# nanoporetech/medaka

Measured on NVIDIA H100. Metric: pileup positions/sec (consensus inference), higher is better.
Workload: dtype f32

## Files before the change

medaka_b200/csrc/gru_wg.cu:

```cuda
#include "common.cuh"
#include "ptx.cuh"
#include "rec_common.cuh"

namespace mdk {

constexpr int RW_THREADS = 256;
constexpr int RW_ABLK = (H / 8) * 64 * 16;
constexpr int RW_XBLK = 2 * 64 * 16;

template <int NT, bool FUSE_X, int OUT>
struct RwCfg {
    static constexpr int N = NT * RT_N;
    static constexpr bool HL = NT == 1;
    static constexpr int ROWS = HL ? 2 * N : N;
    static constexpr int PLANES = HL ? 1 : 2;
    static constexpr int KG = ROWS * 16 + 16;
    static constexpr int HPLANE = (H / 8) * KG;
    static constexpr int XPLANE = 2 * KG;
    static constexpr int HLO = HL ? N * 16 : HPLANE;
    static constexpr int XLO = HL ? N * 16 : XPLANE;
    static constexpr int RED = (RW_THREADS / 32) * NCLS * N;
    static constexpr int wlo_off = 0;
    static constexpr int wxlo_off = wlo_off + 6 * RW_ABLK;
    static constexpr int h_off = wxlo_off + (FUSE_X ? 6 * RW_XBLK : 0);
    static constexpr int x_off = h_off + 2 * PLANES * HPLANE;
    static constexpr int red_off = x_off + (FUSE_X ? 2 * PLANES * XPLANE : 0);
    static constexpr int total = red_off + (OUT == OUT_LOGITS ? 2 * RED * 4 : 0);
    static_assert(total <= 227 * 1024, "smem budget");
};

__device__ __forceinline__ uint32_t ld_u32(const __half *p) { return *reinterpret_cast<const uint32_t *>(p); }

template <int NT, bool FUSE_X, int OUT>
__global__ void __launch_bounds__(RW_THREADS, 1)
rec_tc_kernel(const float *__restrict__ gi, RecX xin, const __half *__restrict__ w_hh, const float *__restrict__ b_hn,
              void *__restrict__ h_out, int64_t B, int64_t T, const float *__restrict__ lin_w,
              float *__restrict__ plog) {
    using L = RwCfg<NT, FUSE_X, OUT>;
    constexpr int N = L::N, NA = N / 2;
    constexpr int NACC = L::ROWS / 2;
    constexpr int NX = FUSE_X ? NACC : NA;
    using MMA = Wgmma<N>;
    using MMA_H = Wgmma<L::ROWS>;
    constexpr bool LOGITS = OUT == OUT_LOGITS;
    extern __shared__ __align__(128) uint8_t smem[];
    const int tid = threadIdx.x, wg = tid >> 7, warp = (tid >> 5) & 3, lane = tid & 31;
    const int gq = lane >> 2, cq = lane & 3;
    const int dir = blockIdx.y;
    const int64_t ntiles = (B + RT_N - 1) / RT_N;
    const int64_t wtile0 = (int64_t)blockIdx.x * NT;
    const int j0 = wg * 64 + warp * 16 + gq;
    const uint32_t sbase = smem_u32(smem);

    for (int i = tid; i < (L::total - L::h_off) / 16; i += RW_THREADS)
        reinterpret_cast<int4 *>(smem + L::h_off)[i] = make_int4(0, 0, 0, 0);
    for (int i = tid; i < 3 * H * (H / 8); i += RW_THREADS) {
        const int kg = i & 15, r = (i >> 4) & (H - 1), gate = i >> 11;
        const uint4 v = *reinterpret_cast<const uint4 *>(w_hh + ((((size_t)dir * 2 + 1) * 3 + gate) * H + r) * H + kg * 8);
        *reinterpret_cast<uint4 *>(smem + L::wlo_off + (gate * 2 + (r >> 6)) * RW_ABLK + kg * 1024 + (r & 63) * 16) = v;
    }
    if (FUSE_X) {
        for (int i = tid; i < 3 * H * 2; i += RW_THREADS) {
            const int kg = i & 1, r = (i >> 1) & (H - 1), gate = i >> 8;
            const uint4 v = *reinterpret_cast<const uint4 *>(xin.w_x + ((((size_t)dir * 2 + 1) * 3 + gate) * H + r) * 16 + kg * 8);
            *reinterpret_cast<uint4 *>(smem + L::wxlo_off + (gate * 2 + (r >> 6)) * RW_XBLK + kg * 1024 + (r & 63) * 16) = v;
        }
    }
    float wlin[2][NCLS];
    if (LOGITS) {
#pragma unroll
        for (int hb = 0; hb < 2; ++hb)
#pragma unroll
            for (int c = 0; c < NCLS; ++c) wlin[hb][c] = lin_w[c * H2 + dir * H + j0 + 8 * hb];
    }
    uint32_t whi[3][H / 16][4];
#pragma unroll
    for (int gate = 0; gate < 3; ++gate)
#pragma unroll
        for (int ks = 0; ks < H / 16; ++ks) {
            const __half *w = w_hh + ((((size_t)dir * 2) * 3 + gate) * H + j0) * H + ks * 16 + 2 * cq;
            whi[gate][ks][0] = ld_u32(w);
            whi[gate][ks][1] = ld_u32(w + 8 * H);
            whi[gate][ks][2] = ld_u32(w + 8);
            whi[gate][ks][3] = ld_u32(w + 8 * H + 8);
        }
    uint32_t wxhi[3][4];
    float bx[3][2] = {};
    if (FUSE_X) {
#pragma unroll
        for (int gate = 0; gate < 3; ++gate) {
            const __half *w = xin.w_x + ((((size_t)dir * 2) * 3 + gate) * H + j0) * 16 + 2 * cq;
            wxhi[gate][0] = ld_u32(w);
            wxhi[gate][1] = ld_u32(w + 8 * 16);
            wxhi[gate][2] = ld_u32(w + 8);
            wxhi[gate][3] = ld_u32(w + 8 * 16 + 8);
            bx[gate][0] = xin.bias[dir * G3 + gate * H + j0];
            bx[gate][1] = xin.bias[dir * G3 + gate * H + j0 + 8];
        }
    }
    const float bhn[2] = {b_hn[dir * H + j0], b_hn[dir * H + j0 + 8]};

    float ar[NACC], az[NACC], an[NACC], axn[NX], hp[NA];
#pragma unroll
    for (int k = 0; k < NA; ++k) hp[k] = 0.f;
    auto load_pre = [&](int64_t t) {
#pragma unroll
        for (int i = 0; i < N / 8; ++i)
#pragma unroll
            for (int hb = 0; hb < 2; ++hb) {
                float2 v[3] = {make_float2(0.f, 0.f), make_float2(0.f, 0.f), make_float2(0.f, 0.f)};
                if (FUSE_X) {
#pragma unroll
                    for (int gate = 0; gate < 3; ++gate) v[gate] = make_float2(bx[gate][hb], bx[gate][hb]);
                } else if (wtile0 + (i >> 1) < ntiles) {
                    const float *p = gi + ((wtile0 + (i >> 1)) * T + t) * GI_TS_FLOATS +
                                     (((dir * 3) * 4 + 2 * (i & 1) + (cq >> 1)) * H + j0 + 8 * hb) * 4 + 2 * (cq & 1);
#pragma unroll
                    for (int gate = 0; gate < 3; ++gate) v[gate] = __ldcs(reinterpret_cast<const float2 *>(p + gate * 16 * H));
                }
                const int k = 4 * i + 2 * hb;
                ar[k] = v[0].x; ar[k + 1] = v[0].y;
                az[k] = v[1].x; az[k + 1] = v[1].y;
                axn[k] = v[2].x; axn[k + 1] = v[2].y;
                an[k] = bhn[hb]; an[k + 1] = bhn[hb];
            }
        if constexpr (L::HL) {
#pragma unroll
            for (int k = NA; k < NACC; ++k) {
                ar[k] = 0.f; az[k] = 0.f; an[k] = 0.f;
                if constexpr (FUSE_X) axn[k] = 0.f;
            }
        }
    };
    const int xF = FUSE_X ? xin.F : 1;
    const float *xsrc[NT];
    int xoff[NT];
    float xreg[NT];
#pragma unroll
    for (int m = 0; m < NT; ++m) {
        const int q = tid + RW_THREADS * m, xn = q / xF, xf = q - xn * xF;
        const bool own = FUSE_X && q < N * xF;
        xoff[m] = own ? (xf >> 3) * L::KG + xn * 16 + (xf & 7) * 2 : -1;
        xsrc[m] = (own && wtile0 * RT_N + xn < B) ? xin.feats + ((wtile0 * RT_N + xn) * T) * xF + xf : nullptr;
        xreg[m] = 0.f;
    }
    auto stage_x = [&](int buf, int m, float v) {
        __half hi, lo;
        split_f16(v, hi, lo);
        *reinterpret_cast<__half *>(smem + L::x_off + buf * L::PLANES * L::XPLANE + xoff[m]) = hi;
        *reinterpret_cast<__half *>(smem + L::x_off + buf * L::PLANES * L::XPLANE + L::XLO + xoff[m]) = lo;
    };
    const int64_t t_first = dir ? T - 1 : 0;
    if (FUSE_X) {
#pragma unroll
        for (int m = 0; m < NT; ++m) {
            if (xoff[m] < 0) continue;
            stage_x(0, m, xsrc[m] ? xsrc[m][t_first * xF] : 0.f);
            if (xsrc[m] && T > 1) xreg[m] = xsrc[m][(dir ? T - 2 : 1) * xF];
        }
    }
    load_pre(t_first);
    fence_proxy_async_smem();
    __syncthreads();

    constexpr int NW = N / 4;
    auto head_partials = [&](int rb) {
        float v[NW][NCLS];
#pragma unroll
        for (int wl = 0; wl < NW; ++wl) {
            const int k = 4 * (wl >> 1) + (wl & 1);
#pragma unroll
            for (int c = 0; c < NCLS; ++c) v[wl][c] = fmaf(wlin[1][c], hp[k + 2], wlin[0][c] * hp[k]);
        }
        int wbase = 0;
#pragma unroll
        for (int lvl = 0; lvl < 3; ++lvl) {
            const int mask = 16 >> lvl;
            const int half = (NW >> lvl) / 2;
            if (half > 0) {
                const bool up = lane & mask;
#pragma unroll
                for (int w = 0; w < NW / 2; ++w) {
                    if (w >= half) continue;
#pragma unroll
                    for (int c = 0; c < NCLS; ++c) {
                        const float send = up ? v[w][c] : v[w + half][c];
                        const float keep = up ? v[w + half][c] : v[w][c];
                        v[w][c] = keep + __shfl_xor_sync(0xffffffffu, send, mask);
                    }
                }
                if (up) wbase += half;
            } else {
#pragma unroll
                for (int c = 0; c < NCLS; ++c) v[0][c] += __shfl_xor_sync(0xffffffffu, v[0][c], mask);
            }
        }
        if (NW >= 8 || !(lane & 4)) {
            float *red = reinterpret_cast<float *>(smem + L::red_off) + rb * L::RED + (tid >> 5) * NCLS * N;
            const int n = 8 * (wbase >> 1) + 2 * cq + (wbase & 1);
#pragma unroll
            for (int c = 0; c < NCLS; ++c) red[c * N + n] = v[0][c];
        }
    };
    auto head_store = [&](int rb, int64_t t) {
        if (tid >= NCLS * N) return;
        const int c = tid / N, n = tid % N;
        const float *red = reinterpret_cast<const float *>(smem + L::red_off) + rb * L::RED + c * N + n;
        float s = red[0];
#pragma unroll
        for (int w = 1; w < RW_THREADS / 32; ++w) s += red[w * NCLS * N];
        const int64_t wt = wtile0 + n / RT_N;
        if (wt < ntiles) plog[((dir * ntiles + wt) * T + t) * PLOG_TS_FLOATS + c * RT_N + (n & 15)] = s;
    };

#pragma unroll 1
    for (int64_t step = 0; step < T; ++step) {
        const int64_t t = dir ? T - 1 - step : step;
        const int buf = (int)(step & 1);
        const uint32_t hb_addr = sbase + L::h_off + buf * L::PLANES * L::HPLANE;
        wg_fence();
        if constexpr (L::HL) {
#pragma unroll
            for (int ks = 0; ks < H / 16; ++ks) {
                const uint64_t bh = make_smem_desc(hb_addr + ks * 2 * L::KG, L::KG, 128);
#pragma unroll
                for (int gate = 0; gate < 3; ++gate) MMA_H::rs(gate == 0 ? ar : (gate == 1 ? az : an), whi[gate][ks], bh, 1u);
#pragma unroll
                for (int gate = 0; gate < 3; ++gate)
                    MMA::ss(gate == 0 ? ar : (gate == 1 ? az : an),
                            make_smem_desc(sbase + L::wlo_off + (gate * 2 + wg) * RW_ABLK + ks * 2 * 1024, 1024, 128), bh, 1u);
            }
        } else {
#pragma unroll
            for (int gate = 0; gate < 3; ++gate) {
                float(&acc)[NACC] = gate == 0 ? ar : (gate == 1 ? az : an);
#pragma unroll
                for (int ks = 0; ks < H / 16; ++ks) {
                    const uint64_t bh = make_smem_desc(hb_addr + ks * 2 * L::KG, L::KG, 128);
                    MMA::rs(acc, whi[gate][ks], bh, 1u);
                    MMA::rs(acc, whi[gate][ks], make_smem_desc(hb_addr + L::HPLANE + ks * 2 * L::KG, L::KG, 128), 1u);
                    MMA::ss(acc, make_smem_desc(sbase + L::wlo_off + (gate * 2 + wg) * RW_ABLK + ks * 2 * 1024, 1024, 128), bh, 1u);
                }
            }
        }
        if constexpr (FUSE_X) {
            const uint32_t xa = sbase + L::x_off + buf * L::PLANES * L::XPLANE;
            const uint64_t bh = make_smem_desc(xa, L::KG, 128);
            if constexpr (L::HL) {
#pragma unroll
                for (int gate = 0; gate < 3; ++gate) MMA_H::rs(gate == 0 ? ar : (gate == 1 ? az : axn), wxhi[gate], bh, 1u);
#pragma unroll
                for (int gate = 0; gate < 3; ++gate)
                    MMA::ss(gate == 0 ? ar : (gate == 1 ? az : axn),
                            make_smem_desc(sbase + L::wxlo_off + (gate * 2 + wg) * RW_XBLK, 1024, 128), bh, 1u);
            } else {
                const uint64_t bl = make_smem_desc(xa + L::XPLANE, L::KG, 128);
#pragma unroll
                for (int gate = 0; gate < 3; ++gate) {
                    float(&acc)[NACC] = gate == 0 ? ar : (gate == 1 ? az : axn);
                    MMA::rs(acc, wxhi[gate], bh, 1u);
                    MMA::rs(acc, wxhi[gate], bl, 1u);
                    MMA::ss(acc, make_smem_desc(sbase + L::wxlo_off + (gate * 2 + wg) * RW_XBLK, 1024, 128), bh, 1u);
                }
            }
        }
        wg_commit();
        if (!FUSE_X && tid == 0 && step + GI_PREFETCH_STEPS < T) {
            const int64_t tp = dir ? t - GI_PREFETCH_STEPS : t + GI_PREFETCH_STEPS;
#pragma unroll
            for (int m = 0; m < NT; ++m) {
                if (wtile0 + m >= ntiles) break;
                const float *blk = gi + ((wtile0 + m) * T + tp) * GI_TS_FLOATS + (int64_t)dir * (GI_TS_FLOATS / 2);
#pragma unroll
                for (int i = 0; i < 12; ++i) bulk_prefetch_l2(blk + i * 512, 2048);
            }
        }
        if (LOGITS && step > 0) {
            if (step > 1) head_store((int)((step - 1) & 1), dir ? t + 2 : t - 2);
            head_partials((int)(step & 1));
        }
        wg_wait_all();
        wg_hold(ar); wg_hold(az); wg_hold(an); wg_hold(axn);

        uint8_t *hw = smem + L::h_off + (buf ^ 1) * L::PLANES * L::HPLANE;
#pragma unroll
        for (int k = 0; k < NA; ++k) {
            float pr = ar[k], pz = az[k], pn = an[k], px = axn[k], r, z;
            if constexpr (L::HL) {
                pr += ar[k + NA]; pz += az[k + NA]; pn += an[k + NA];
                if constexpr (FUSE_X) px += axn[k + NA];
                const float a = 1.f + ex2_approx(fminf(pr, EXP_CLAMP)), b = 1.f + ex2_approx(fminf(pz, EXP_CLAMP));
                const float q = rcp_approx(a * b);
                r = b * q;
                z = a * q;
            } else {
                r = rcp_approx(1.f + ex2_approx(fminf(pr, EXP_CLAMP)));
                z = rcp_approx(1.f + ex2_approx(fminf(pz, EXP_CLAMP)));
            }
            const float en = ex2_approx(fminf(fmaf(r, pn, px), EXP_CLAMP));
            const float n = (en - 1.f) * rcp_approx(en + 1.f);
            hp[k] = fmaf(z, hp[k] - n, n);
            const int j = j0 + 8 * ((k >> 1) & 1), col = 8 * (k >> 2) + 2 * cq + (k & 1);
            __half hi, lo;
            split_f16(hp[k], hi, lo);
            *reinterpret_cast<__half *>(hw + (j >> 3) * L::KG + col * 16 + (j & 7) * 2) = hi;
            *reinterpret_cast<__half *>(hw + L::HLO + (j >> 3) * L::KG + col * 16 + (j & 7) * 2) = lo;
        }
        if (FUSE_X && step + 1 < T) {
#pragma unroll
            for (int m = 0; m < NT; ++m) {
                if (xoff[m] < 0) continue;
                stage_x(buf ^ 1, m, xreg[m]);
                if (xsrc[m] && step + 2 < T) xreg[m] = xsrc[m][(dir ? t - 2 : t + 2) * xF];
            }
        }
        if (!LOGITS) {
#pragma unroll
            for (int k = 0; k < NA; ++k) {
                const int i = k >> 2, n = 8 * i + 2 * cq + (k & 1);
                const int64_t wt = wtile0 + (i >> 1);
                if (wt >= ntiles) continue;
                const int64_t orow = (wt * T + t) * RT_N + (n & 15);
                const int kcol = dir * H + j0 + 8 * ((k >> 1) & 1);
                if (OUT == OUT_TILES) {
                    __half hi, lo;
                    split_f16(hp[k], hi, lo);
                    __half *o = reinterpret_cast<__half *>(reinterpret_cast<uint8_t *>(h_out) + (orow >> 7) * (int64_t)XT_TILE_BYTES +
                                                           (kcol >> 3) * (XT_ROWS * 16) + (orow & (XT_ROWS - 1)) * 16) + (kcol & 7);
                    o[0] = hi;
                    o[XT_PLANE_BYTES / 2] = lo;
                } else {
                    reinterpret_cast<float *>(h_out)[orow * H2 + kcol] = hp[k];
                }
            }
        }
        if (step + 1 < T) load_pre(dir ? t - 1 : t + 1);
        fence_proxy_async_smem();
        __syncthreads();
    }
    if (LOGITS) {
        if (T > 1) head_store((int)((T - 1) & 1), dir ? 1 : T - 2);
        head_partials((int)(T & 1));
        __syncthreads();
        head_store((int)(T & 1), dir ? 0 : T - 1);
    }
}

template <int NT, bool FX, int OUT>
static cudaError_t launch_rec(const float *gi, const RecX &xin, const __half *w_hh_tm, const float *b_hn, void *out,
                              const float *lin_w, int64_t B, int64_t T, cudaStream_t s) {
    auto kern = rec_tc_kernel<NT, FX, OUT>;
    constexpr int smem_bytes = RwCfg<NT, FX, OUT>::total;
    cudaError_t e = cudaFuncSetAttribute(kern, cudaFuncAttributeMaxDynamicSharedMemorySize, smem_bytes);
    if (e != cudaSuccess) return e;
    const int64_t tiles = (B + RT_N - 1) / RT_N;
    dim3 grid((unsigned)((tiles + NT - 1) / NT), NDIR);
    constexpr bool LOGITS = OUT == OUT_LOGITS;
    kern<<<grid, RW_THREADS, smem_bytes, s>>>(gi, xin, w_hh_tm, b_hn, LOGITS ? nullptr : out, B, T, lin_w,
                                              LOGITS ? static_cast<float *>(out) : nullptr);
    return cudaGetLastError();
}

template <int NT>
static cudaError_t launch_rec_nt(const float *gi, const RecX *xin, const __half *w_hh_tm, const float *b_hn, int out_kind,
                                 void *out, const float *lin_w, int64_t B, int64_t T, cudaStream_t s) {
    if (xin)
        return out_kind == OUT_TILES ? launch_rec<NT, true, OUT_TILES>(gi, *xin, w_hh_tm, b_hn, out, nullptr, B, T, s)
                                     : cudaErrorInvalidValue;
    const RecX none{nullptr, nullptr, nullptr, 0};
    switch (out_kind) {
    case OUT_TILES: return launch_rec<NT, false, OUT_TILES>(gi, none, w_hh_tm, b_hn, out, nullptr, B, T, s);
    case OUT_ROWS: return launch_rec<NT, false, OUT_ROWS>(gi, none, w_hh_tm, b_hn, out, nullptr, B, T, s);
    case OUT_LOGITS:
        return lin_w ? launch_rec<NT, false, OUT_LOGITS>(gi, none, w_hh_tm, b_hn, out, lin_w, B, T, s) : cudaErrorInvalidValue;
    }
    return cudaErrorInvalidValue;
}

cudaError_t launch_rec_tc(const float *gi, const RecX *xin, const __half *w_hh_tm, const float *b_hn, int tiles_per_cta,
                          int out_kind, void *out, const float *lin_w, int64_t B, int64_t T, cudaStream_t s) {
    if (B == 0 || T == 0) return cudaSuccess;
    switch (tiles_per_cta) {
    case 1: return launch_rec_nt<1>(gi, xin, w_hh_tm, b_hn, out_kind, out, lin_w, B, T, s);
    case 2: return launch_rec_nt<2>(gi, xin, w_hh_tm, b_hn, out_kind, out, lin_w, B, T, s);
    }
    return cudaErrorInvalidValue;
}

constexpr int GW_THREADS = 256;
constexpr int GW_QK = 8;
constexpr int GW_STAGE_PLANE = GW_QK * XT_ROWS * 16;
constexpr int GW_STAGE = 2 * GW_STAGE_PLANE;
constexpr int GW_NQ = XT_K / 8 / GW_QK;
constexpr int GW_KS = XT_K / 16;
constexpr int GW_TS = XT_ROWS / WT;
constexpr int GW_QUAD = H * 4;
constexpr int GW_QUAD_PAD = GW_QUAD + 16;
constexpr int GW_OUT_OFF = GW_NQ * GW_STAGE;
constexpr int GW_BAR_OFF = GW_OUT_OFF + GW_TS * 4 * GW_QUAD_PAD * 4;
constexpr int GW_SMEM = GW_BAR_OFF + 2 * GW_NQ * 8;
static_assert(GW_SMEM <= 227 * 1024, "smem budget");
static_assert(GW_TS * 4 == 32, "one bulk store per lane of warp 0");

__global__ void __launch_bounds__(GW_THREADS, 1)
gemm_tc_kernel(const uint8_t *__restrict__ x_tiles, const __half *__restrict__ w_in_tm, const float *__restrict__ bias,
               float *__restrict__ gi, int64_t P, int64_t ntiles) {
    extern __shared__ __align__(128) uint8_t smem[];
    uint64_t *full = reinterpret_cast<uint64_t *>(smem + GW_BAR_OFF), *empty = full + GW_NQ;
    float *stg = reinterpret_cast<float *>(smem + GW_OUT_OFF);
    const int tid = threadIdx.x, wg = tid >> 7, warp = (tid >> 5) & 3, lane = tid & 31;
    const int gq = lane >> 2, cq = lane & 3;
    const int blk = blockIdx.x;
    const int j0 = wg * 64 + warp * 16 + gq;
    const uint32_t sbase = smem_u32(smem);
    const int64_t my_tiles = blockIdx.y < ntiles ? (ntiles - 1 - blockIdx.y) / gridDim.y + 1 : 0;
    auto issue = [&](int64_t n, int q) {
        const uint8_t *src = x_tiles + (blockIdx.y + n * gridDim.y) * (int64_t)XT_TILE_BYTES + q * GW_STAGE_PLANE;
        mbar_arrive_expect_tx(&full[q], GW_STAGE);
        bulk_g2s(smem + q * GW_STAGE, src, GW_STAGE_PLANE, &full[q]);
        bulk_g2s(smem + q * GW_STAGE + GW_STAGE_PLANE, src + XT_PLANE_BYTES, GW_STAGE_PLANE, &full[q]);
    };
    if (tid == 0) {
        for (int q = 0; q < GW_NQ; ++q) {
            mbar_init(&full[q], 1);
            mbar_init(&empty[q], GW_THREADS / 32);
        }
        fence_mbar_init();
        if (my_tiles > 0)
            for (int q = 0; q < GW_NQ; ++q) issue(0, q);
    }
    uint32_t wa[2][GW_KS][4];
#pragma unroll
    for (int p = 0; p < 2; ++p)
#pragma unroll
        for (int ks = 0; ks < GW_KS; ++ks) {
            const __half *w = w_in_tm + (((size_t)blk * 2 + p) * H + j0) * H2 + ks * 16 + 2 * cq;
            wa[p][ks][0] = ld_u32(w);
            wa[p][ks][1] = ld_u32(w + 8 * H2);
            wa[p][ks][2] = ld_u32(w + 8);
            wa[p][ks][3] = ld_u32(w + 8 * H2 + 8);
        }
    const float bj[2] = {bias[blk * H + j0], bias[blk * H + j0 + 8]};
    const uint64_t policy = l2_evict_first_policy();
    __syncthreads();
    auto release = [&](int64_t n, int q) {
        if (lane == 0) mbar_arrive(&empty[q]);
        if (tid == 0 && n + 1 < my_tiles) {
            mbar_wait(&empty[q], (uint32_t)(n & 1));
            issue(n + 1, q);
        }
        __syncwarp();
    };
    float acc[64];
#pragma unroll 1
    for (int64_t n = 0; n < my_tiles; ++n) {
#pragma unroll
        for (int q = 0; q < GW_NQ; ++q) {
            mbar_wait(&full[q], (uint32_t)(n & 1));
            wg_fence();
#pragma unroll
            for (int prod = 0; prod < 3; ++prod) {
                const int pa = prod == 2, pb = prod == 1;
#pragma unroll
                for (int kk = 0; kk < GW_QK / 2; ++kk) {
                    const uint64_t b = make_smem_desc(sbase + q * GW_STAGE + pb * GW_STAGE_PLANE + 2 * kk * (XT_ROWS * 16),
                                                      XT_ROWS * 16, 128);
                    Wgmma<128>::rs(acc, wa[pa][q * (GW_QK / 2) + kk], b, (q | prod | kk) ? 1u : 0u);
                }
            }
            wg_commit();
            if (q > 0) {
                wg_wait_1();
                release(n, q - 1);
            }
        }
        wg_wait_all();
        wg_hold(acc);
        release(n, GW_NQ - 1);

        const int64_t tile = blockIdx.y + n * gridDim.y;
        const int64_t prem = P - tile * XT_ROWS;
        if (tid < 32) bulk_wait_read_all();
        __syncthreads();
#pragma unroll
        for (int k = 0; k < 64; k += 2) {
            const int i = k >> 2, hb = (k >> 1) & 1;
            float *o = stg + ((i >> 1) * 4 + 2 * (i & 1) + (cq >> 1)) * GW_QUAD_PAD + (j0 + 8 * hb) * 4 + 2 * (cq & 1);
            *reinterpret_cast<float2 *>(o) = make_float2(acc[k] + bj[hb], acc[k + 1] + bj[hb]);
        }
        fence_proxy_async_smem();
        __syncthreads();
        if (tid < 32) {
            const int ts = lane >> 2, cg = lane & 3;
            if (ts * WT < prem)
                bulk_s2g(gi + (((tile * GW_TS + ts) * 6 + blk) * 4 + cg) * GW_QUAD, stg + lane * GW_QUAD_PAD,
                         GW_QUAD * 4, policy);
            bulk_commit();
        }
    }
    if (tid < 32) bulk_wait_all();
}

cudaError_t launch_gemm_tc(const void *x_tiles, const __half *w_in_tm, const float *bias, float *gi, int64_t P,
                           int sm_count, cudaStream_t s) {
    if (P == 0) return cudaSuccess;
    const int64_t ntiles = (P + XT_ROWS - 1) / XT_ROWS;
    cudaError_t ea = cudaFuncSetAttribute(gemm_tc_kernel, cudaFuncAttributeMaxDynamicSharedMemorySize, GW_SMEM);
    if (ea != cudaSuccess) return ea;
    int64_t ct = sm_count / 6;
    if (ct < 1) ct = 1;
    if (ct > ntiles) ct = ntiles;
    dim3 grid(6, (unsigned)ct);
    gemm_tc_kernel<<<grid, GW_THREADS, GW_SMEM, s>>>(reinterpret_cast<const uint8_t *>(x_tiles), w_in_tm, bias, gi, P, ntiles);
    return cudaGetLastError();
}

__global__ void __launch_bounds__(256, 1)
selftest_kernel(const float *__restrict__ A, const float *__restrict__ Bm, float *__restrict__ D, int N, int K) {
    extern __shared__ __align__(128) uint8_t smem[];
    const int a_plane = 128 * K * 2, b_plane = N * K * 2;
    uint8_t *sa = smem, *sb = smem + 2 * a_plane;
    const int tid = threadIdx.x, wg = tid >> 7, warp = (tid >> 5) & 3, lane = tid & 31;
    for (int i = tid; i < 128 * K; i += 256) {
        const int r = i / K, k = i % K;
        __half hi, lo;
        split_f16(A[i], hi, lo);
        const int off = (k / 8) * (128 * 16) + r * 16 + (k % 8) * 2;
        *reinterpret_cast<__half *>(sa + off) = hi;
        *reinterpret_cast<__half *>(sa + a_plane + off) = lo;
    }
    for (int i = tid; i < N * K; i += 256) {
        const int r = i / K, k = i % K;
        __half hi, lo;
        split_f16(Bm[i], hi, lo);
        const int off = (k / 8) * (N * 16) + r * 16 + (k % 8) * 2;
        *reinterpret_cast<__half *>(sb + off) = hi;
        *reinterpret_cast<__half *>(sb + b_plane + off) = lo;
    }
    fence_proxy_async_smem();
    __syncthreads();
    for (int n0 = 0; n0 < N; n0 += 16) {
        float d[8];
        wg_fence();
        uint32_t acc = 0;
        for (int prod = 0; prod < 3; ++prod) {
            const int pa = (prod == 2), pb = (prod == 1);
            for (int ks = 0; ks < K / 16; ++ks) {
                const uint64_t ad = make_smem_desc(smem_u32(sa + pa * a_plane) + ks * 2 * 128 * 16 + wg * 64 * 16, 128 * 16, 128);
                const uint64_t bd = make_smem_desc(smem_u32(sb + pb * b_plane) + ks * 2 * N * 16 + n0 * 16, N * 16, 128);
                Wgmma<16>::ss(d, ad, bd, acc);
                acc = 1;
            }
        }
        wg_commit();
        wg_wait_all();
        wg_hold(d);
        const int row = wg * 64 + warp * 16 + (lane >> 2);
        for (int k = 0; k < 8; ++k)
            D[(row + 8 * ((k >> 1) & 1)) * N + n0 + 8 * (k >> 2) + 2 * (lane & 3) + (k & 1)] = d[k];
    }
}

int selftest_umma(int device, const float *A, const float *B, float *D, int N, int K, int variant) {
    MDK_REQUIRE(N >= 16 && N <= 128 && N % 16 == 0, MDK_ERR_ARG, "selftest_umma: N must be a multiple of 16 in [16,128]");
    MDK_REQUIRE(K >= 16 && K <= 256 && K % 16 == 0, MDK_ERR_ARG, "selftest_umma: K must be a multiple of 16 in [16,256]");
    MDK_REQUIRE(variant == 0, MDK_ERR_ARG, "selftest_umma: variant must be 0");
    MDK_CUDA(cudaSetDevice(device));
    float *dA = nullptr, *dB = nullptr, *dD = nullptr;
    MDK_CUDA(cudaMalloc(&dA, sizeof(float) * 128 * K));
    MDK_CUDA(cudaMalloc(&dB, sizeof(float) * N * K));
    MDK_CUDA(cudaMalloc(&dD, sizeof(float) * 128 * N));
    MDK_CUDA(cudaMemcpy(dA, A, sizeof(float) * 128 * K, cudaMemcpyHostToDevice));
    MDK_CUDA(cudaMemcpy(dB, B, sizeof(float) * N * K, cudaMemcpyHostToDevice));
    const int smem = 2 * 128 * K * 2 + 2 * N * K * 2;
    MDK_REQUIRE(smem <= 227 * 1024, MDK_ERR_ARG, "selftest_umma: N*K too large for shared memory");
    MDK_CUDA(cudaFuncSetAttribute(selftest_kernel, cudaFuncAttributeMaxDynamicSharedMemorySize, smem));
    selftest_kernel<<<1, 256, smem>>>(dA, dB, dD, N, K);
    MDK_CUDA(cudaGetLastError());
    MDK_CUDA(cudaDeviceSynchronize());
    MDK_CUDA(cudaMemcpy(D, dD, sizeof(float) * 128 * N, cudaMemcpyDeviceToHost));
    cudaFree(dA); cudaFree(dB); cudaFree(dD);
    return MDK_OK;
}

}
```

Baseline: 162.0 million.

## Store tiled hidden outputs from shared memory with vector writes overlapped with MMA

OUT_TILES hidden-state output is no longer written as scattered per-element half stores after the gate math. The previous step's staged hi/lo h tiles are now copied from shared memory with 16-byte vector stores while the recurrent MMAs are in flight. The x-feature prefetch moves to right after the MMA commit, and the gi address computation is hoisted into a per-thread base pointer with a simplified bound check. This cuts per-step store instruction count and moves global latency off the serial critical path. The cost is some extra shared memory reads and more complex index bookkeeping.

```diff
diff --git a/medaka_b200/csrc/gru_wg.cu b/medaka_b200/csrc/gru_wg.cu
--- a/medaka_b200/csrc/gru_wg.cu
+++ b/medaka_b200/csrc/gru_wg.cu
@@ -103,6 +103,8 @@
     float ar[NACC], az[NACC], an[NACC], axn[NX], hp[NA];
 #pragma unroll
     for (int k = 0; k < NA; ++k) hp[k] = 0.f;
+    const float *gi_thr = FUSE_X ? nullptr
+                                 : gi + wtile0 * T * GI_TS_FLOATS + ((dir * 3 * 4 + (cq >> 1)) * H + j0) * 4 + 2 * (cq & 1);
     auto load_pre = [&](int64_t t) {
 #pragma unroll
         for (int i = 0; i < N / 8; ++i)
@@ -112,9 +114,8 @@
                 if (FUSE_X) {
 #pragma unroll
                     for (int gate = 0; gate < 3; ++gate) v[gate] = make_float2(bx[gate][hb], bx[gate][hb]);
-                } else if (wtile0 + (i >> 1) < ntiles) {
-                    const float *p = gi + ((wtile0 + (i >> 1)) * T + t) * GI_TS_FLOATS +
-                                     (((dir * 3) * 4 + 2 * (i & 1) + (cq >> 1)) * H + j0 + 8 * hb) * 4 + 2 * (cq & 1);
+                } else if (i < 2 || wtile0 + (i >> 1) < ntiles) {
+                    const float *p = gi_thr + ((i >> 1) * T + t) * GI_TS_FLOATS + (2 * (i & 1) * H + 8 * hb) * 4;
 #pragma unroll
                     for (int gate = 0; gate < 3; ++gate) v[gate] = __ldcs(reinterpret_cast<const float2 *>(p + gate * 16 * H));
                 }
@@ -156,7 +157,6 @@
         for (int m = 0; m < NT; ++m) {
             if (xoff[m] < 0) continue;
             stage_x(0, m, xsrc[m] ? xsrc[m][t_first * xF] : 0.f);
-            if (xsrc[m] && T > 1) xreg[m] = xsrc[m][(dir ? T - 2 : 1) * xF];
         }
     }
     load_pre(t_first);
@@ -212,6 +212,19 @@
         const int64_t wt = wtile0 + n / RT_N;
         if (wt < ntiles) plog[((dir * ntiles + wt) * T + t) * PLOG_TS_FLOATS + c * RT_N + (n & 15)] = s;
     };
+    auto store_h0 = [&](int b, int64_t t) {
+#pragma unroll
+        for (int r = 0; r < NT * 512 / RW_THREADS; ++r) {
+            const int q = tid + RW_THREADS * r, row = q & 15, kg = (q >> 4) & 15, p = (q >> 8) & 1, m = q >> 9;
+            const int64_t wt = wtile0 + m;
+            if (wt >= ntiles) continue;
+            const int64_t orow = (wt * T + t) * RT_N + row;
+            const int4 v = *reinterpret_cast<const int4 *>(smem + L::h_off + b * L::PLANES * L::HPLANE + p * L::HLO + kg * L::KG +
+                                                           (m * RT_N + row) * 16);
+            *reinterpret_cast<int4 *>(reinterpret_cast<uint8_t *>(h_out) + (orow >> 7) * (int64_t)XT_TILE_BYTES +
+                                      p * XT_PLANE_BYTES + (dir * (H / 8) + kg) * (XT_ROWS * 16) + (orow & (XT_ROWS - 1)) * 16) = v;
+        }
+    };
 
 #pragma unroll 1
     for (int64_t step = 0; step < T; ++step) {
@@ -265,6 +278,12 @@
             }
         }
         wg_commit();
+        if (FUSE_X && step + 1 < T) {
+#pragma unroll
+            for (int m = 0; m < NT; ++m)
+                if (xsrc[m]) xreg[m] = xsrc[m][(dir ? t - 1 : t + 1) * xF];
+        }
+        if (OUT == OUT_TILES && step > 0) store_h0(buf, dir ? t + 1 : t - 1);
         if (!FUSE_X && tid == 0 && step + GI_PREFETCH_STEPS < T) {
             const int64_t tp = dir ? t - GI_PREFETCH_STEPS : t + GI_PREFETCH_STEPS;
 #pragma unroll
@@ -311,33 +330,23 @@
             for (int m = 0; m < NT; ++m) {
                 if (xoff[m] < 0) continue;
                 stage_x(buf ^ 1, m, xreg[m]);
-                if (xsrc[m] && step + 2 < T) xreg[m] = xsrc[m][(dir ? t - 2 : t + 2) * xF];
-            }
-        }
-        if (!LOGITS) {
+            }
+        }
+        if (OUT == OUT_ROWS) {
 #pragma unroll
             for (int k = 0; k < NA; ++k) {
                 const int i = k >> 2, n = 8 * i + 2 * cq + (k & 1);
                 const int64_t wt = wtile0 + (i >> 1);
                 if (wt >= ntiles) continue;
                 const int64_t orow = (wt * T + t) * RT_N + (n & 15);
-                const int kcol = dir * H + j0 + 8 * ((k >> 1) & 1);
-                if (OUT == OUT_TILES) {
-                    __half hi, lo;
-                    split_f16(hp[k], hi, lo);
-                    __half *o = reinterpret_cast<__half *>(reinterpret_cast<uint8_t *>(h_out) + (orow >> 7) * (int64_t)XT_TILE_BYTES +
-                                                           (kcol >> 3) * (XT_ROWS * 16) + (orow & (XT_ROWS - 1)) * 16) + (kcol & 7);
-                    o[0] = hi;
-                    o[XT_PLANE_BYTES / 2] = lo;
-                } else {
-                    reinterpret_cast<float *>(h_out)[orow * H2 + kcol] = hp[k];
-                }
-            }
-        }
-        if (step + 1 < T) load_pre(dir ? t - 1 : t + 1);
+                reinterpret_cast<float *>(h_out)[orow * H2 + dir * H + j0 + 8 * ((k >> 1) & 1)] = hp[k];
+            }
+        }
+        if (FUSE_X || step + 1 < T) load_pre(dir ? t - 1 : t + 1);
         fence_proxy_async_smem();
         __syncthreads();
     }
+    if (OUT == OUT_TILES) store_h0((int)(T & 1), dir ? 0 : T - 1);
     if (LOGITS) {
         if (T > 1) head_store((int)((T - 1) & 1), dir ? 1 : T - 2);
         head_partials((int)(T & 1));
```

Measured after the change: 168.3 million (median of 6 runs). 1.04x the previous value.
